# zotya701/OpenCL_Path_tracer

Measured on AMD Instinct MI355X. Metric: Msamples/s (whole node) at 1920x1080, 8-bounce Cornell box, higher is better.
Workload: dtype f32

## Files before the change

### opencl_path_tracer_amd/csrc/pt_builder.cpp

```cpp
#include "pt_context.hpp"

namespace ptamd {

struct RefOrder {
    const std::vector<pt_triangle>& tris;
    std::vector<int32_t>& rank;
    int32_t& next_rank;
    bool degenerate = false;

    struct Range { int32_t begin, end, depth; };

    static int32_t split(const Range& r, int32_t* idx, int32_t* tmp, const float* cx, const float* cy, const float* cz) {
        const int32_t n = r.end - r.begin;
        if (n <= 6) return 0;
        int32_t* ix = idx + r.begin;
        float mx = cx[ix[0]], my = cy[ix[0]], mz = cz[ix[0]];
        for (int32_t i = 1; i < n; ++i) {
            mx = mx + cx[ix[i]];
            my = my + cy[ix[i]];
            mz = mz + cz[ix[i]];
        }
        const float m[3] = {mx / (float)(unsigned long)n, my / (float)(unsigned long)n, mz / (float)(unsigned long)n};
        const float* c[3] = {cx, cy, cz};
        int axis = r.depth % 3;
// ... 978 lines not shown
                    else {
                        const int32_t first = (~ref) >> 3, count = ((~ref) & 7) + 1;
                        good = good && first >= nf && first + count <= n;
                    }
                }
            }
            if (!good) ok.store(false);
        });
        if (!ok.load()) { drop(); return fail(ctx, PT_EHIP, "internal: the device SAH builder returned a malformed tree"); }
    }
    (void)hipFree(r.d_orig);
    r.d_orig = nullptr;
    ctx->host_packets_stale = true;
    ctx->bvh_depth = sah ? r.depth : r.depth + 1;
    ctx->n_flat = nf;
    clk.lap("download + list in front");
    const bool retopped = !sah && sah_top_rebuild(ctx, ctx->lbvh_cluster);
    clk.lap("SAH top over clusters");
    bool wide_done = false;
    int rc = plan_node_placement(ctx, retopped ? nullptr : r.d_nodes, &wide_done);
    clk.lap("node placement + 4-wide nodes");
    if (rc != PT_OK) { drop(); return rc; }
    if (retopped) ctx->bvh_depth = ctx->interior_depth + 1;
    if (ctx->d_tris) (void)hipFree(ctx->d_tris);
    if (ctx->d_meta) (void)hipFree(ctx->d_meta);
    ctx->d_tris = r.d_tris;
    ctx->d_meta = r.d_meta;
    if (retopped) {
        (void)hipFree(r.d_nodes);
        if ((rc = upload_vec(ctx, &ctx->d_nodes, ctx->nodes.data(), sizeof(Node64) * ctx->nodes.size())) != PT_OK) return rc;
    } else {
        if (ctx->d_nodes) (void)hipFree(ctx->d_nodes);
        ctx->d_nodes = r.d_nodes;
        if (ctx->treelet_nodes > 0) PT_HIP(ctx, hipMemcpy(ctx->d_nodes, ctx->nodes.data(), sizeof(Node64) * ctx->nodes.size(), hipMemcpyHostToDevice));
    }
    if (!wide_done && (rc = upload_vec(ctx, &ctx->d_nodes4, ctx->nodes4.data(), sizeof(Node4q) * ctx->nodes4.size())) != PT_OK) return rc;
    if ((rc = alloc_stack_overflow(ctx)) != PT_OK) return rc;
    clk.lap("uploads");
    *done = true;
    return PT_OK;
}

static void compute_cost_boxes(pt_context* ctx) { compute_cost_boxes_impl(ctx); }

int pt_upload_triangles(pt_context* ctx) {
    if (!ctx) return PT_EINVAL;
// ... 8 lines not shown
        int rcd = build_on_device(ctx, &done);
        if (rcd != PT_OK) return rcd;
        if (done) {
            compute_cost_boxes(ctx);
            ctx->bvh_build_ms = std::chrono::duration<double, std::milli>(std::chrono::steady_clock::now() - t0).count();
            ctx->bvh_on_device = 1;
            ctx->tris_uploaded = true;
            return PT_OK;
        }
    }
    ctx->bvh_on_device = 0;
    ctx->host_packets_stale = false;
    int rc = build_and_pack(ctx);
    if (rc != PT_OK) return rc;
    PhaseClock clk("pt_upload_triangles");
    if ((rc = plan_node_placement(ctx)) != PT_OK) return rc;
    clk.lap("node placement + 4-wide nodes");
    ctx->bvh_build_ms = std::chrono::duration<double, std::milli>(std::chrono::steady_clock::now() - t0).count();
    if (ctx->has_device) {
        PT_HIP(ctx, hipSetDevice(ctx->device));
        if ((rc = upload_vec(ctx, &ctx->d_nodes, ctx->nodes.data(), sizeof(Node64) * ctx->nodes.size())) != PT_OK) return rc;
        if ((rc = upload_vec(ctx, &ctx->d_nodes4, ctx->nodes4.data(), sizeof(Node4q) * ctx->nodes4.size())) != PT_OK) return rc;
        if ((rc = alloc_stack_overflow(ctx)) != PT_OK) return rc;
        if ((rc = upload_vec(ctx, &ctx->d_tris, ctx->packets.data(), sizeof(TriPacket) * ctx->packets.size())) != PT_OK) return rc;
        if ((rc = upload_vec(ctx, &ctx->d_meta, ctx->meta.data(), sizeof(TriMeta) * ctx->meta.size())) != PT_OK) return rc;
        clk.lap("device allocations + copies");
    }
    ctx->tris_uploaded = true;
    return PT_OK;
}


}
```

### opencl_path_tracer_amd/csrc/pt_context.hpp

```cpp
#pragma once

#include "pt_internal.hpp"

#include <algorithm>
#include <atomic>
#include <chrono>
#include <cmath>
#include <condition_variable>
#include <functional>
#include <mutex>
#include <cstdio>
#include <cstring>
#include <limits>
#include <memory>
#include <numeric>
#include <queue>
#include <thread>

using namespace ptamd;

namespace ptamd {
struct EventPair {
    hipEvent_t a = nullptr, b = nullptr;
};
// ... 23 lines not shown
    bool tris_uploaded = false, mats_uploaded = false;

    std::vector<Node64> nodes;
    std::vector<Node4q> nodes4;
    int wide_pending = 0;
    std::vector<TriPacket> packets;
    bool host_packets_stale = false;
    std::vector<TriMeta> meta;
    std::vector<int32_t> orig;
    int bvh_depth = 0;
    int interior_depth = 0;
    int n_flat = 0;
    int n_fbox = 0;
    uint8_t fbox_rep[32] = {};
    uint32_t fbox_mask[32] = {};

    float4* d_nodes = nullptr;
    float4* d_nodes4 = nullptr;
    uint32_t* d_stack_ovf = nullptr;
    size_t stack_ovf_lanes = 0;
    float4* d_tris = nullptr;
    TriMeta* d_meta = nullptr;
    pt_material* d_mats = nullptr;
    int32_t* d_rnds = nullptr;
    float4* d_colors = nullptr;
    pt_ray* d_rays = nullptr;
    float4* d_ldr = nullptr;
    unsigned long long* d_stats = nullptr;
    float4* d_wf_state = nullptr;
    int32_t* d_wf_queues = nullptr;
    std::vector<float> cost_boxes;
    uint32_t* d_wf_counters = nullptr;
    hipStream_t wf_stream[kWfMaxChains] = {};
    hipEvent_t wf_event[kWfMaxChains] = {};
    int poll_timeout_ms = 10000;
    int debug_stall_tile = -1;
    bool counters_suspect = false;
    bool launched_since_check = false;
    int wf_streams = -1;
    bool own_rnds = true, own_colors = true;
    hipStream_t stream = nullptr;

    int32_t current_sample = 0;

    int variant = 0;
    int lds_scene = 2;
// ... 199 lines not shown
};

template <class F>
void parallel_for(size_t n, size_t grain, int threads, F fn) {
    const size_t nt = std::min<size_t>((size_t)std::max(threads, 1), (n + grain - 1) / std::max<size_t>(grain, 1));
    if (nt <= 1) { fn((size_t)0, n); return; }
    const size_t per = (n + nt - 1) / nt;
    HostPool::get().run(nt, (int)nt, [&](size_t k) {
        const size_t b = k * per, e = std::min(n, b + per);
        if (b < e) fn(b, e);
    });
}
int deepest_interior_node(const std::vector<Node64>& nodes);
int reindex_treelet(std::vector<Node64>& nodes, int interior_depth, int want);

int32_t count_local_rows(int32_t H, int32_t rank, int32_t world, int32_t rb);
int wide_stack_entries(int pending);
int stack_entries_for(int interior_depth);
bool whole_tree_fits_lds(size_t n_nodes, size_t n_tris, int interior_depth, int n_flat);
int plan_node_placement(pt_context* ctx, const float4* d_bvh2 = nullptr, bool* wide_on_device = nullptr);
int alloc_stack_overflow(pt_context* ctx);
int seed_upload(pt_context* ctx, const int32_t* global_seeds);
void fill_params(const pt_context* ctx, const pt_camera* cam, RenderParams* p);
int check_ready(pt_context* ctx, const pt_camera* cam);
int time_begin(pt_context* ctx, EventPair** ep);
int time_end(pt_context* ctx, EventPair* ep);
int time_collect(pt_context* ctx);
int sync_and_check(pt_context* ctx);
inline int32_t local_tiles(const pt_context* c) { return ((c->W + 7) / 8) * ((c->local_rows + 7) / 8); }
template <class T>
int upload_vec(pt_context* ctx, T** dptr, const void* src, size_t bytes) {
    if (*dptr) { PT_HIP(ctx, hipFree(*dptr)); *dptr = nullptr; }
    PT_HIP(ctx, hipMalloc((void**)dptr, std::max<size_t>(bytes, 64)));
    if (bytes < 64) PT_HIP(ctx, hipMemset(*dptr, 0, 64));
    if (bytes) PT_HIP(ctx, hipMemcpy(*dptr, src, bytes, hipMemcpyHostToDevice));
    return PT_OK;
}


}
```

### opencl_path_tracer_amd/csrc/pt_device.hpp

```cpp
#pragma once

#include "pt_internal.hpp"

#include <algorithm>

#ifndef PT_GLOBAL_SLAB_FMA
#define PT_GLOBAL_SLAB_FMA 1
#endif
#ifndef PT_WIDE_STEP_V1
#define PT_WIDE_STEP_V1 0
#endif
#ifndef PT_PHASE_SWITCH_GLOBAL
#define PT_PHASE_SWITCH_GLOBAL 1
#endif
#ifndef PT_PHASE_SWITCH_LDS
#define PT_PHASE_SWITCH_LDS 1
#endif
#ifndef PT_WIDE_PREDICATED_STORES
#define PT_WIDE_PREDICATED_STORES 1
#endif

namespace ptamd {

struct f3 {
// ... 716 lines not shown
        }
    }
    template <bool COUNT>
    PT_DEV void leaf_step(const SceneView& sv, WorkCount* wc) {
        const int popped = stack_get(sv, tos);
        const int v = leaf_bits(cur);
        const int first = v >> 3, count = (v & 7) + 1;
        for (int j = 0; j < count; ++j) tri_step<COUNT>(sv, first + j, wc);
        cur = popped;
        tos -= stride;
    }
};

template <int MODE, bool COUNT>
PT_DEV int closest_hit(const SceneView& sv, f3 P, f3 D, const LaneStack<typename StackOf<MODE>::type> stk, float* t_out, WorkCount* wc) {
    Trav<MODE> tr;
    tr.begin(P, D, stk);
    tr.template flat_pass<COUNT>(sv, wc);
    while (!tr.done()) tr.template round<COUNT>(sv, wc);
    *t_out = tr.best_t;
    return tr.best;
}

template <bool SK>
PT_DEV f3 diffuse_direction(f3 N, float rnd1, float rnd2) {
    const float E = 0.001f;
    const bool yaxis = __builtin_fabsf(N.x) <= E && __builtin_fabsf(N.z) <= E;
    const float other = yaxis ? N.y : N.x;
    const float l2 = fmaf_(N.z, N.z, other * other);
    float rl, r, z;
    if (wave_all(rsqrt_window(l2) && rnd1 >= kSqrtWindowLo && rnd1 < 1.0f)) {
        rl = rsqrt_core(l2);
        r = sqrt_core(rnd1);
        z = sqrt_core(1.0f - rnd1);
    } else {
        rl = 1.0f / __builtin_sqrtf(l2);
        r = __builtin_sqrtf(rnd1);
        z = __builtin_sqrtf(1.0f - rnd1);
    }
    const f3 Z = yaxis ? mk(0.0f, -N.z * rl, N.y * rl) : mk(-N.z * rl, 0.0f, N.x * rl);
    const f3 X = cross3(N, Z);
    const float theta = (float)(6.283185307179586 * (double)rnd2);
    float sn, cs;
    spec_sincos<SK>(theta, &sn, &cs);
    const float x = r * cs, y = r * sn;
    f3 d = X * x;
    d = madd(N, z, d);
    d = madd(Z, y, d);
    return d;
}

PT_DEV f3 fresnel(f3 F0, f3 N, f3 D) {
    const float cosa = __builtin_fabsf(dot3(N, D));
    const float p5 = spec_pow5(1.0f - cosa);
    return mk(fmaf_(1.0f - F0.x, p5, F0.x), fmaf_(1.0f - F0.y, p5, F0.y), fmaf_(1.0f - F0.z, p5, F0.z));
}

struct PathRegs {
    f3 fL, fB, fS, fR, color;
    PT_DEV void reset() {
        fL = mk(1.f, 1.f, 1.f);
        fB = fL;
        fS = fL;
        fR = fL;
        color = mk(0.f, 0.f, 0.f);
    }
    PT_DEV f3 L() const { return fL; }
    PT_DEV f3 B() const { return fB; }
    PT_DEV f3 S() const { return fS; }
    PT_DEV f3 R() const { return fR; }
    PT_DEV f3 C() const { return color; }
    PT_DEV void setL(f3 v) { fL = v; }
    PT_DEV void setB(f3 v) { fB = v; }
    PT_DEV void setS(f3 v) { fS = v; }
    PT_DEV void setR(f3 v) { fR = v; }
    PT_DEV void setC(f3 v) { color = v; }
};

struct NoShadeHook {
    static constexpr bool active = false;
};

template <bool SK, class ST, class HOOK = NoShadeHook>
PT_DEV void shade_hit(f3& rP, f3& rD, ST& st, int& seed, bool& inside, const RenderParams& p, const float4* tris, const TriMeta* meta, int ti, float t,
                      HOOK* hook = nullptr) {
    const float4 c = tris[ti * 3 + 2];
    f3 N = mk(c.y, c.z, c.w);
    const f3 hp = madd(rD, t, rP);
    const pt_material* __restrict__ m = &p.mats[meta[ti].mati];
    const int type = m->type;
    if (p.iterations == 1) st.setC(ldf3(m->kd) + ldf3(m->emission));
    if (dot3(rD, N) > 0.0f) N = -N;
    const bool lobe = type == 0 || type == 3, spec = type == 1 || type == 2;
    f3 dnew = rD;
    float side = 0.001f;
    float inten = 0.0f;
    float wb = 1.0f;
    if (lobe) {
        inten = max0(dot3(-rD, N));
        if constexpr (HOOK::active) {
            if (type == 3) wb = hook->emitter_weight(ti, t, inten, rD);
            hook->light_sample(st, p, m, type, N, hp);
        }
        const float rnd1 = lcg_rand(seed), rnd2 = lcg_rand(seed);
        dnew = diffuse_direction<SK>(N, rnd1, rnd2);
    } else if (spec) {
        const f3 oldD = rD;
        const f3 F0 = ldf3(m->F0);
        const f3 F = fresnel(F0, N, oldD);
        dnew = oldD - (N * dot3(N, oldD)) * 2.0f;
        if (type == 2) {
            float n = m->n;
            if (inside) n = 1.0f / n;
            const float rnd = lcg_rand(seed);
            const float cosa = dot3(-oldD, N);
            const float disc = 1.0f - (fmaf_(-cosa, cosa, 1.0f) / n) / n;
            const float prob = ((F.x + F.y) + F.z) / 3.0f;
            const bool refr = disc > 0.0f && rnd > prob;
            if (refr) {
                const f3 dn = mk(oldD.x / n, oldD.y / n, oldD.z / n);
                dnew = madd(N, cosa / n - sqrt_rn(disc), dn);
                const float k = 1.0f / (1.0f - prob);
                st.setR((st.R() * mk(1.0f - F.x, 1.0f - F.y, 1.0f - F.z)) * k);
                inside = !inside;
                side = -0.001f;
            } else {
                const float k = 1.0f / prob;
                st.setR((st.R() * F) * k);
            }
        } else {
            st.setS(st.S() * F);
        }
    }
    if (lobe || spec) {
        rD = normalize3(dnew);
        rP = madd(N, side, hp);
    }
    if (type == 0) {
        const float idiff = max0(dot3(rD, N));
        st.setL(st.L() * (ldf3(m->kd) * idiff));
        float pw = 1.0f;
        if (!m->_pad) {
            const f3 view = normalize3(ldf3(p.cam.eye) - hp);
            const f3 halfway = normalize3(view + rD);
            const float ispec = max0(dot3(N, halfway));
            pw = spec_pow<SK>(ispec, m->shininess);
        }
        st.setB(st.B() * (ldf3(m->ks) * pw));
    } else if (type == 3) {
        const f3 e = ((ldf3(m->emission) * (st.L() + st.B())) * st.S()) * st.R();
        if constexpr (HOOK::active) st.setC(madd(e * wb, inten, st.C()));
        else st.setC(madd(e, inten, st.C()));
    }
    if constexpr (HOOK::active) hook->end_vertex(lobe, N);
}

PT_DEV f3 running_mean(f3 acc, f3 color, int s) {
    const float cs = (float)s, cs1 = (float)(s + 1);
    return mk(fmaf_(acc.x, cs, color.x) / cs1, fmaf_(acc.y, cs, color.y) / cs1, fmaf_(acc.z, cs, color.z) / cs1);
}

PT_DEV float luminance(f3 c) { return fmaf_(0.0722f, c.z, fmaf_(0.7152f, c.y, 0.2126f * c.x)); }
PT_DEV float running_moment(float m2, f3 color, int s) {
    const float l = luminance(color);
    return fmaf_(m2, (float)s, l * l) / (float)(s + 1);
}


PT_DEV unsigned stage_ref(float slot) {
    const int r = __float_as_int(slot);
    return (unsigned)(r < 0 ? (0x8000 | ~r) : r) & 0xffffu;
// ... 122 lines not shown
```

### opencl_path_tracer_amd/csrc/pt_host.cpp

```cpp
#include "pt_context.hpp"

namespace {
thread_local std::string g_create_error;
}

namespace ptamd {

int fail(pt_context* ctx, int code, const std::string& msg) {
    if (ctx) ctx->err = msg; else g_create_error = msg;
    return code;
}

int host_threads(const pt_context* ctx) {
    const unsigned hw = std::thread::hardware_concurrency();
    return ctx->build_threads > 0 ? ctx->build_threads : (int)std::min(16u, std::max(1u, hw));
}

int fail_ctx(pt_context* ctx, int code, const std::string& msg) { return fail(ctx, code, msg); }
int append_triangles(pt_context* ctx, int64_t n, pt_triangle** tail) {
    if (!ctx || n < 0 || !tail) return PT_EINVAL;
    if ((int64_t)ctx->tris.size() + n > kMaxTriangles) return fail(ctx, PT_EINVAL, "more than 2^26 triangles");
    const size_t old = ctx->tris.size();
    ctx->tris.resize(old + (size_t)n);
    ctx->tris_uploaded = false;
// ... 153 lines not shown
        pt_destroy(ctx);
        return fail(nullptr, rc, msg);
    }
    *out = ctx;
    return PT_OK;
}

int pt_create(int device, int32_t width, int32_t height, pt_context** out) {
    return pt_create_tiled(device, width, height, 0, 1, 8, out);
}

void pt_destroy(pt_context* ctx) {
    if (!ctx) return;
    if (ctx->has_device) {
        (void)hipSetDevice(ctx->device);
        (void)hipDeviceSynchronize();
        for (auto& e : ctx->events) { if (e.a) (void)hipEventDestroy(e.a); if (e.b) (void)hipEventDestroy(e.b); }
        if (ctx->d_nodes) (void)hipFree(ctx->d_nodes);
        if (ctx->d_nodes4) (void)hipFree(ctx->d_nodes4);
        if (ctx->d_stack_ovf) (void)hipFree(ctx->d_stack_ovf);
        if (ctx->d_tris) (void)hipFree(ctx->d_tris);
        if (ctx->d_meta) (void)hipFree(ctx->d_meta);
        if (ctx->d_mats) (void)hipFree(ctx->d_mats);
        if (ctx->d_rays) (void)hipFree(ctx->d_rays);
        if (ctx->d_ldr) (void)hipFree(ctx->d_ldr);
        if (ctx->d_stats) (void)hipFree(ctx->d_stats);
        if (ctx->d_tile_counter) (void)hipFree(ctx->d_tile_counter);
        if (ctx->d_tile_done) (void)hipFree(ctx->d_tile_done);
        if (ctx->d_tile_cost) (void)hipFree(ctx->d_tile_cost);
        if (ctx->d_adapt_snap) (void)hipFree(ctx->d_adapt_snap);
        if (ctx->d_adapt_spp) (void)hipFree(ctx->d_adapt_spp);
        if (ctx->d_adapt_err) (void)hipFree(ctx->d_adapt_err);
        if (ctx->d_adapt_active) (void)hipFree(ctx->d_adapt_active);
        if (ctx->d_adapt_list) (void)hipFree(ctx->d_adapt_list);
        if (ctx->h_adapt_count) (void)hipHostFree(ctx->h_adapt_count);
        if (ctx->d_aov) (void)hipFree(ctx->d_aov);
        if (ctx->d_dn) (void)hipFree(ctx->d_dn);
        if (ctx->d_variance) (void)hipFree(ctx->d_variance);
        if (ctx->d_temporal) (void)hipFree(ctx->d_temporal);
        if (ctx->d_temporal_var) (void)hipFree(ctx->d_temporal_var);
        if (ctx->d_nee_tri) (void)hipFree(ctx->d_nee_tri);
        if (ctx->d_nee_cdf) (void)hipFree(ctx->d_nee_cdf);
        if (ctx->d_nee_pdf_area) (void)hipFree(ctx->d_nee_pdf_area);
        if (ctx->d_env_texels) (void)hipFree(ctx->d_env_texels);
        if (ctx->d_env_row_cdf) (void)hipFree(ctx->d_env_row_cdf);
        if (ctx->d_env_col_cdf) (void)hipFree(ctx->d_env_col_cdf);
// ... 31 lines not shown

int pt_add_triangle(pt_context* ctx, const pt_triangle* t) { return pt_add_triangles(ctx, t, 1); }

int pt_add_triangles(pt_context* ctx, const pt_triangle* t, int64_t n) {
    if (!ctx || (!t && n) || n < 0) return PT_EINVAL;
    if ((int64_t)ctx->tris.size() + n > kMaxTriangles)
        return fail(ctx, PT_EINVAL, "more than 2^26 triangles");
    ctx->tris.insert(ctx->tris.end(), t, t + n);
    ctx->tris_uploaded = false;
    return PT_OK;
}

int pt_upload_materials(pt_context* ctx) {
    if (!ctx) return PT_EINVAL;
    ctx->aov_valid = false;
    ctx->nee_valid = false;
    for (const pt_triangle& t : ctx->tris)
        if (t.mati >= ctx->mats.size()) return fail(ctx, PT_EINVAL, "a triangle references a material index that was never added");
    if (ctx->has_device) {
        PT_HIP(ctx, hipSetDevice(ctx->device));
        std::vector<pt_material> dm(ctx->mats);
        for (pt_material& m : dm)
            m._pad = (m.ks.s[0] == 0.0f && m.ks.s[1] == 0.0f && m.ks.s[2] == 0.0f && std::isfinite(m.shininess) && m.shininess >= 0.0f) ? 1 : 0;
        int rc = upload_vec(ctx, &ctx->d_mats, dm.data(), sizeof(pt_material) * dm.size());
        if (rc != PT_OK) return rc;
    }
    ctx->mats_uploaded = true;
    return PT_OK;
}

int pt_seed_default(pt_context* ctx) {
    PT_NEED_DEVICE(ctx);
    const size_t n = (size_t)ctx->W * (size_t)ctx->H;
    std::vector<int32_t> g(n);
    uint64_t x = 1;
    for (size_t i = 0; i < n; ++i) {
        x = (x * 16807ull) % 2147483647ull;
        g[i] = (int32_t)x;
    }
    return seed_upload(ctx, g.data());
}

int pt_upload_seeds(pt_context* ctx, const int32_t* seeds, int64_t n) {
    PT_NEED_DEVICE(ctx);
    if (!seeds || n != (int64_t)ctx->W * ctx->H) return fail(ctx, PT_EINVAL, "seeds must hold width*height ints (global frame)");
    return seed_upload(ctx, seeds);
}

// ... 887 lines not shown
```

### opencl_path_tracer_amd/csrc/pt_internal.hpp

```cpp
#pragma once

#include <hip/hip_runtime.h>

#include <atomic>
#include <chrono>
#include <cstdint>
#include <cstdio>
#include <cstdlib>
#include <string>
#include <vector>

#include "pt_api.h"

namespace ptamd {

struct Node64 {
    float q[3][4];
    int32_t left, right;
    int32_t pad[2];
};
static_assert(sizeof(Node64) == 64, "Node64 must be 64 B");

struct TriPacket {
    float v[12];
};
static_assert(sizeof(TriPacket) == 48, "TriPacket must be 48 B");

struct TriMeta {
    int32_t rank;
    int32_t mati;
};

struct Node4q {
    float origin[3];
    uint8_t exp[3];
    uint8_t nchild;
    uint32_t qlo_x, qhi_x, qlo_y, qhi_y;
    uint32_t qlo_z, qhi_z;
    uint32_t spare[2];
    int32_t ref[4];
};
static_assert(sizeof(Node4q) == 64, "Node4q must be 64 B");
constexpr int32_t kWideNoChild = ~0;
constexpr int kWideLdsEntries = 20;
bool build_wide_nodes(const std::vector<Node64>& bvh2, std::vector<Node4q>* out, int* max_pending, int threads);

enum : int { kNodesLds = 0, kNodesGlobal = 1, kNodesTreelet = 2, kNodesWide = 3 };

constexpr int64_t kMaxTriangles = (int64_t)1 << 26;

constexpr int64_t kDeviceBuildFrom = 16384;
constexpr int kMaxLeaf = 4;
constexpr int kMaxDepth = 30;
constexpr int kTileCounterError = 16;
// ... 31 lines not shown
    int32_t n_flat;
    int32_t n_fbox;
    uint8_t fbox_rep[32];
    uint32_t fbox_mask[32];
    int32_t node_mode;
    int32_t treelet_nodes;
    int32_t stack_entries;
    uint32_t* stack_ovf;
    int32_t stack_ovf_lanes;
    uint32_t* tile_counter;
    uint32_t poll_ticks;
    int32_t debug_stall_tile;
    int32_t n_tiles;
    int32_t n_taper;
    uint16_t taper_end[kMaxTaperPasses];
    int32_t chunk_spp;
    uint32_t* tile_done;
    int32_t suspend_lanes;
    int32_t node_min_lanes;
    int32_t leaf_min_lanes;
    int32_t migrate_lanes;
    uint32_t* tile_cost;
    const int32_t* tile_list;
    int32_t moments;
};

template <class P>
__host__ __device__ __forceinline__ int global_row(const P& p, int lrow) {
    return ((lrow / p.rows_per_block) * p.world + p.rank) * p.rows_per_block + lrow % p.rows_per_block;
}

constexpr int kWfCounterStride = 8;
constexpr int kWfMaxBounces = 1023;
constexpr int kWfGenRow = 0;
__host__ __device__ inline int wf_row(int bounce) { return bounce == 0 ? kWfGenRow : bounce + 1; }
constexpr int kWfMaxCostBoxes = 8;
constexpr int kWfMaxChains = 8;
constexpr int kWfDefaultChains = 4;
enum : int { kWfL = 0, kWfB = 1, kWfS = 2, kWfR = 3, kWfC = 4, kWfFields = 5, kWfInsideBit = 1 << 5, kWfBZeroBit = 1 << 6 };
struct WfParams {
    RenderParams rp;
    float* sP;
    float4* rsA[2][2];
    float4* rsB[2][2];
    float4* rsC[2][2];
    float2* hit[2];
// ... 76 lines not shown
    return n;
}

struct PhaseClock {
    const char* who;
    const bool on = std::getenv("PTAMD_TRACE") != nullptr;
    std::chrono::steady_clock::time_point t0 = std::chrono::steady_clock::now();
    explicit PhaseClock(const char* w) : who(w) {}
    void lap(const char* what) {
        if (!on) return;
        const auto t1 = std::chrono::steady_clock::now();
        std::fprintf(stderr, "[%s] %-32s %8.1f ms\n", who, what, std::chrono::duration<double, std::milli>(t1 - t0).count());
        t0 = t1;
    }
};

int traversal_block(int node_mode, bool wide_lds_block);
size_t traversal_lds_bytes(const RenderParams& p, int block);
hipError_t launch_gen_ray(const RenderParams& p, hipStream_t stream);
hipError_t launch_trace_ray(const RenderParams& p, const LaunchConfig& lc, hipStream_t stream);
hipError_t launch_render_mega(const RenderParams& p, const LaunchConfig& lc, hipStream_t stream);
hipError_t launch_resolve_reinhard(const float4* colors, float4* out, int64_t n, hipStream_t stream);
hipError_t launch_filt_im(const float4* colors, float4* out, int32_t width, int32_t height, hipStream_t stream);
hipError_t launch_wf_generate(const WfParams& p, hipStream_t stream);
hipError_t launch_wf_intersect(const WfParams& p, int bounce, int cu_count, hipStream_t stream);
hipError_t launch_wf_shade(const WfParams& p, int bounce, hipStream_t stream);
hipError_t launch_adaptive_tiles(const float4* colors, float4* snap, const int32_t* list, int32_t n_list, int32_t width, int32_t rows, int mode,
                                 float threshold, int32_t spp, float* tile_err, int32_t* tile_spp, uint8_t* active, hipStream_t stream);
hipError_t launch_compact_tiles(const uint8_t* active, int32_t n, int32_t* list, int32_t* count, hipStream_t stream);
hipError_t launch_debug_closest_hit(const RenderParams& p, const pt_ray* rays, int64_t n, float* out_t, int32_t* out_tri, int cu_count, hipStream_t stream);
hipError_t launch_debug_math(int fn, unsigned long long first, unsigned long long n, unsigned long long* out, uint32_t* bad, long long bad_cap, int cu_count,
                             hipStream_t stream);
hipError_t launch_aovs(const RenderParams& p, int32_t subpixels, int32_t specular_depth, int64_t npix, float4* albedo_rgbm, float4* normal_depth,
                       int cu_count, hipStream_t stream);
struct AtrousStep {
    int32_t step;
    int32_t demodulate;
    int32_t color_on, normal_on, depth_on;
    float color_scale;
    float sigma_color2, sigma_normal, sigma_depth;
};
hipError_t launch_atrous(const float4* in, float4* out, const float4* albedo, const float4* nd, int32_t W, int32_t H, const AtrousStep& s,
                         bool first, bool last, hipStream_t stream);
struct AtrousVarStep {
    int32_t step;
    int32_t demodulate;
// ... 95 lines not shown
```

### opencl_path_tracer_amd/csrc/pt_kernels.hip

```cpp
#include "pt_device.hpp"


#include <algorithm>

namespace ptamd {

__global__ void __launch_bounds__(256) k_gen_ray(RenderParams p) {
    const PixelId px = pixel_of_thread(p);
    if (px.li < 0) return;
    int seed = p.rnds[px.li];
    const float rnd1 = lcg_rand(seed), rnd2 = lcg_rand(seed);
    f3 P, D;
    camera_get_ray(px.gid, p.cam, rnd1, rnd2, &P, &D);
    p.rnds[px.li] = seed;
    float4* r = reinterpret_cast<float4*>(&p.rays[px.li]);
    r[0] = make_float4(P.x, P.y, P.z, 0.0f);
    r[1] = make_float4(D.x, D.y, D.z, 0.0f);
}

enum : int { kSchedLockstep = 0, kSchedSuspend = 1, kSchedMigrate = 2 };


PT_DEV void fold_sample(const RenderParams& p, int li, f3 color, int s) {
    f3 acc = mk(0.0f, 0.0f, 0.0f);
    float m2 = 0.0f;
    if (s != 0) {
        const float4 c = p.colors[li];
        acc = mk(c.x, c.y, c.z);
        m2 = c.w;
    }
    acc = running_mean(acc, color, s);
    m2 = p.moments ? running_moment(m2, color, s) : 0.0f;
    p.colors[li] = make_float4(acc.x, acc.y, acc.z, m2);
}

template <bool SPLIT, int MODE, bool COUNT, bool LEAN, bool SK>
PT_DEV void render_pixel_lockstep(const RenderParams& p, const SceneView& sv, const LaneStack<typename StackOf<MODE>::type> stk, const PixelId px,
                                  int s_begin, int s_end, unsigned* segs, WorkCount* wc) {
    int seed = p.rnds[px.li];
    f3 acc = mk(0.0f, 0.0f, 0.0f);
    float m2 = 0.0f;
    if (!LEAN && s_begin != 0) {
        const float4 c = p.colors[px.li];
        acc = mk(c.x, c.y, c.z);
// ... 265 lines not shown
            }
            cur_item = -1;
            if (nxt_item < 0 && !no_more) {
                nxt_item = fetch();
                no_more = __builtin_amdgcn_readfirstlane((int)(nxt_item < 0));
                nxt_ready = 0;
            }
            if (nxt_item < 0) break;
            if (!nxt_ready) {
                if (!wait_released(nxt_item)) break;
                if (pass_of(nxt_item) > 0) __builtin_amdgcn_fence(__ATOMIC_ACQUIRE, "agent");
            }
            cur_item = __builtin_amdgcn_readfirstlane(nxt_item);
            cur_end = __builtin_amdgcn_readfirstlane(end_of(nxt_item));
            nxt_item = -1;
            nxt_ready = 0;
            if (on_next) on_next = false;
            else take_pixel(cur_item);
        } else if (__popcll(__ballot(parked && !on_next)) >= p.migrate_lanes) {
            if (nxt_item < 0 && !no_more) {
                nxt_item = fetch();
                no_more = __builtin_amdgcn_readfirstlane((int)(nxt_item < 0));
                nxt_ready = 0;
                nxt_end = __builtin_amdgcn_readfirstlane(end_of(nxt_item));
            }
            if (nxt_item >= 0 && !nxt_ready && released(nxt_item)) {
                if (pass_of(nxt_item) > 0) __builtin_amdgcn_fence(__ATOMIC_ACQUIRE, "agent");
                nxt_ready = 1;
            }
            if (nxt_item >= 0 && nxt_ready && parked && !on_next) {
                on_next = true;
                take_pixel(nxt_item);
            }
        }
        if (!parked && fresh && !traversing) {
            st.reset();
            inside = false;
            const float rnd1 = lcg_rand(seed), rnd2 = lcg_rand(seed);
            camera_get_ray_xy((float)(pxy & 0xffffu), (float)(pxy >> 16), p.cam, rnd1, rnd2, &rP, &rD);
            bounce = 0;
            fresh = false;
        }
        bool finished = !parked;
        if (!parked && (traversing || bounce < p.iterations)) {
            tr.setup(rP, rD);
            if (!traversing) {
                tr.restart(stk);
                tr.template flat_pass<COUNT>(sv, wc);
            }
            for (;;) {
                if (COUNT && first_active_lane()) wc->wrounds++;
                tr.template round<COUNT>(sv, wc);
                const unsigned long long unfinished = __ballot(!tr.done());
                if (unfinished == 0) break;
                if (__popcll(unfinished) <= p.suspend_lanes && __ballot(tr.done()) != 0) break;
            }
            traversing = !tr.done();
            if (traversing) {
                finished = false;
            } else {
                ++my_segs;
                if (tr.best >= 0) {
                    if (COUNT) { if (first_active_lane()) wc->wshade++; count_low(wc, 3); }
                    shade_hit<SK>(rP, rD, st, seed, inside, p, sv.tris, sv.meta, tr.best, tr.best_t);
                    ++bounce;
                    finished = (bounce >= p.iterations);
                }
            }
        }
        samples += (unsigned long long)__popcll(__ballot(finished));
        if (finished) {
            if (LEAN) fold_sample(p, li, st.C(), s);
            else {
                acc = running_mean(acc, st.C(), s);
                if (p.moments) m2 = running_moment(m2, st.C(), s);
            }
            ++s;
            fresh = true;
        }
    }
    {
        unsigned v = my_segs;
        for (int off = 32; off > 0; off >>= 1) v += __shfl_down(v, off, 64);
        *segs_tot += (unsigned)__builtin_amdgcn_readfirstlane((int)v);
        *samples_tot += samples;
    }
    if (COUNT) {
// ... 257 lines not shown
```

### opencl_path_tracer_amd/csrc/pt_launch.cpp

```cpp
#include "pt_context.hpp"

namespace ptamd {

int32_t count_local_rows(int32_t H, int32_t rank, int32_t world, int32_t rb) {
    int32_t n = 0;
    for (int32_t r = 0; r < H; ++r)
        if ((r / rb) % world == rank) ++n;
    return n;
}

int wide_stack_entries(int pending) { return ((pending + 4) + 1) & ~1; }
int stack_entries_for(int interior_depth) { return std::min(kStackEntries, ((interior_depth + 2) + 1) & ~1); }


bool whole_tree_fits_lds(size_t n_nodes, size_t n_tris, int interior_depth, int n_flat) {
    const bool s16 = n_nodes <= 32767 && n_tris <= 4096;
    const size_t block = (size_t)kLdsBlockBase;
    return s16 && (size_t)kLdsNodeBytes * n_nodes + 16 + (size_t)stack_entries_for(interior_depth) * 2 * block + (size_t)n_flat * 100 + 64 <= kLdsPerCu / 2;
}

static void group_flat_boxes(pt_context* ctx) {
    ctx->n_fbox = 0;
    float ext[32][6];
    for (int k = 0; k < ctx->n_flat; ++k) {
// ... 114 lines not shown
        }
    }
    if (!ctx->nodes4.empty() && (p->node_mode == kNodesGlobal || ctx->wide_nodes == 2)) {
        p->node_mode = kNodesWide;
        p->treelet_nodes = 0;
        p->nodes = ctx->d_nodes4;
        p->stack_entries = std::min(ctx->wide_lds_entries, wide_stack_entries(ctx->wide_pending));
        p->stack_ovf = ctx->d_stack_ovf;
        p->stack_ovf_lanes = (int32_t)ctx->stack_ovf_lanes;
    }
    p->tile_counter = nullptr;
    p->poll_ticks = (uint32_t)std::min<int64_t>((int64_t)ctx->poll_timeout_ms * 100000, 0xffffffffll);
    p->debug_stall_tile = ctx->debug_stall_tile;
    p->chunk_spp = 0;
    p->n_taper = 0;
    p->tile_done = nullptr;
    p->n_tiles = ((ctx->W + 7) / 8) * ((ctx->local_rows + 7) / 8);
    p->suspend_lanes = ctx->suspend_lanes >= 0 ? ctx->suspend_lanes : (p->node_mode == kNodesLds ? 16 : 24);
    p->node_min_lanes = ctx->node_min_lanes >= 0 ? ctx->node_min_lanes : (p->node_mode == kNodesLds ? 3 : 6);
    p->leaf_min_lanes = ctx->leaf_min_lanes >= 0 ? ctx->leaf_min_lanes : 4;
    p->migrate_lanes = ctx->migrate_lanes > 0 ? ctx->migrate_lanes : 1;
}

int check_ready(pt_context* ctx, const pt_camera* cam) {
    if (!cam) return fail(ctx, PT_EINVAL, "camera is NULL");
    if (!ctx->tris_uploaded) return fail(ctx, PT_EINVAL, "pt_upload_triangles has not been called");
    if (!ctx->mats_uploaded) return fail(ctx, PT_EINVAL, "pt_upload_materials has not been called");
    if ((int32_t)cam->XM != ctx->W || (int32_t)cam->YM != ctx->H)
        return fail(ctx, PT_EINVAL, "camera XM/YM do not match the context's frame size");
    return PT_OK;
}

int time_begin(pt_context* ctx, EventPair** ep) {
    *ep = nullptr;
    if (!ctx->timing) return PT_OK;
    if (ctx->events_used == ctx->events.size()) {
        EventPair e;
        PT_HIP(ctx, hipEventCreate(&e.a));
        PT_HIP(ctx, hipEventCreate(&e.b));
        ctx->events.push_back(e);
    }
    *ep = &ctx->events[ctx->events_used++];
    PT_HIP(ctx, hipEventRecord((*ep)->a, ctx->stream));
    return PT_OK;
}
int time_end(pt_context* ctx, EventPair* ep) {
// ... 199 lines not shown
            }
        if (ctx->timing && ctx->events_used >= 4096) {
            int rc = time_collect(ctx);
            if (rc != PT_OK) return rc;
        }
    }
    for (int c = 1; c < chains; ++c) {
        PT_HIP(ctx, hipEventRecord(ctx->wf_event[c], ctx->wf_stream[c]));
        PT_HIP(ctx, hipStreamWaitEvent(ctx->stream, ctx->wf_event[c], 0));
    }
    return PT_OK;
}

static int launch_megakernel(pt_context* ctx, RenderParams& p, const int32_t* tile_list, int32_t n_active) {
    int rc = PT_OK;
    const int32_t nsamples = p.nsamples;
    if (tile_list) {
        p.tile_list = tile_list;
        p.n_tiles = n_active;
    }
    const size_t frame_tiles = (size_t)local_tiles(ctx);
    LaunchConfig lc;
    launch_cfg(ctx, p, &lc);
    if (ctx->persistent) {
        if (int rc2 = prepare_work_counter(ctx)) return rc2;
        p.tile_counter = ctx->d_tile_counter;
        const int resident_waves = ptamd_resident_waves(ctx, lc);
        const int auto_chunk = auto_chunk_spp(p.n_tiles, resident_waves, nsamples, lc.schedule, p.node_mode);
        const int chunk = ctx->chunk_spp >= 0 ? ctx->chunk_spp : auto_chunk;
        int n_pass = chunk > 0 ? (int)(((int64_t)nsamples + chunk - 1) / chunk) : 1;
        const int taper = ctx->chunk_taper >= 0 ? ctx->chunk_taper : auto_chunk_taper(nsamples, lc.schedule, p.node_mode);
        if (chunk > 0 && nsamples > chunk && taper > 0 && taper < chunk && nsamples < 65536) {
            std::vector<int> ends;
            int done = 0;
            while (nsamples - done > chunk) { done += chunk; ends.push_back(done); }
            for (int left = nsamples - done; left > 0;) {
                const int take = left >= 2 * taper ? left / 2 : left;
                done += take;
                left -= take;
                ends.push_back(done);
            }
            if ((int)ends.size() <= kMaxTaperPasses) {
                n_pass = p.n_taper = (int)ends.size();
                for (int k = 0; k < n_pass; ++k) p.taper_end[k] = (uint16_t)ends[k];
            }
        }
// ... 200 lines not shown
```

Baseline: 2779.

## Precompute per-triangle shade records with normal, material fields and tangent frames

```diff
diff --git a/opencl_path_tracer_amd/csrc/pt_builder.cpp b/opencl_path_tracer_amd/csrc/pt_builder.cpp
--- a/opencl_path_tracer_amd/csrc/pt_builder.cpp
+++ b/opencl_path_tracer_amd/csrc/pt_builder.cpp
@@ -1024,6 +1024,7 @@
     clk.lap("node placement + 4-wide nodes");
     if (rc != PT_OK) { drop(); return rc; }
     if (retopped) ctx->bvh_depth = ctx->interior_depth + 1;
+    ctx->shaderec_dirty = true;
     if (ctx->d_tris) (void)hipFree(ctx->d_tris);
     if (ctx->d_meta) (void)hipFree(ctx->d_meta);
     ctx->d_tris = r.d_tris;
@@ -1078,6 +1079,7 @@
         if ((rc = upload_vec(ctx, &ctx->d_nodes, ctx->nodes.data(), sizeof(Node64) * ctx->nodes.size())) != PT_OK) return rc;
         if ((rc = upload_vec(ctx, &ctx->d_nodes4, ctx->nodes4.data(), sizeof(Node4q) * ctx->nodes4.size())) != PT_OK) return rc;
         if ((rc = alloc_stack_overflow(ctx)) != PT_OK) return rc;
+        ctx->shaderec_dirty = true;
         if ((rc = upload_vec(ctx, &ctx->d_tris, ctx->packets.data(), sizeof(TriPacket) * ctx->packets.size())) != PT_OK) return rc;
         if ((rc = upload_vec(ctx, &ctx->d_meta, ctx->meta.data(), sizeof(TriMeta) * ctx->meta.size())) != PT_OK) return rc;
         clk.lap("device allocations + copies");
diff --git a/opencl_path_tracer_amd/csrc/pt_context.hpp b/opencl_path_tracer_amd/csrc/pt_context.hpp
--- a/opencl_path_tracer_amd/csrc/pt_context.hpp
+++ b/opencl_path_tracer_amd/csrc/pt_context.hpp
@@ -69,6 +69,10 @@
     float4* d_tris = nullptr;
     TriMeta* d_meta = nullptr;
     pt_material* d_mats = nullptr;
+    ShadeRec* d_shaderec = nullptr;
+    size_t shaderec_cap = 0;
+    bool shaderec_dirty = true;
+    int32_t mats_on_device = 0;
     int32_t* d_rnds = nullptr;
     float4* d_colors = nullptr;
     pt_ray* d_rays = nullptr;
@@ -314,6 +318,7 @@
 int alloc_stack_overflow(pt_context* ctx);
 int seed_upload(pt_context* ctx, const int32_t* global_seeds);
 void fill_params(const pt_context* ctx, const pt_camera* cam, RenderParams* p);
+int ensure_shade_records(pt_context* ctx, RenderParams* p);
 int check_ready(pt_context* ctx, const pt_camera* cam);
 int time_begin(pt_context* ctx, EventPair** ep);
 int time_end(pt_context* ctx, EventPair* ep);
diff --git a/opencl_path_tracer_amd/csrc/pt_device.hpp b/opencl_path_tracer_amd/csrc/pt_device.hpp
--- a/opencl_path_tracer_amd/csrc/pt_device.hpp
+++ b/opencl_path_tracer_amd/csrc/pt_device.hpp
@@ -762,12 +762,36 @@
     return tr.best;
 }
 
+PT_DEV float frame_l2(f3 N, bool* yaxis) {
+    const float E = 0.001f;
+    *yaxis = __builtin_fabsf(N.x) <= E && __builtin_fabsf(N.z) <= E;
+    const float other = *yaxis ? N.y : N.x;
+    return fmaf_(N.z, N.z, other * other);
+}
+PT_DEV void frame_from_rl(f3 N, bool yaxis, float rl, f3* Z, f3* X) {
+    *Z = yaxis ? mk(0.0f, -N.z * rl, N.y * rl) : mk(-N.z * rl, 0.0f, N.x * rl);
+    *X = cross3(N, *Z);
+}
+PT_DEV void tangent_frame(f3 N, f3* Z, f3* X) {
+    bool yaxis;
+    const float l2 = frame_l2(N, &yaxis);
+    frame_from_rl(N, yaxis, rsqrt_rn(l2), Z, X);
+}
+template <bool SK>
+PT_DEV f3 lobe_direction(f3 N, f3 Z, f3 X, float r, float z, float rnd2) {
+    const float theta = (float)(6.283185307179586 * (double)rnd2);
+    float sn, cs;
+    spec_sincos<SK>(theta, &sn, &cs);
+    const float x = r * cs, y = r * sn;
+    f3 d = X * x;
+    d = madd(N, z, d);
+    d = madd(Z, y, d);
+    return d;
+}
 template <bool SK>
 PT_DEV f3 diffuse_direction(f3 N, float rnd1, float rnd2) {
-    const float E = 0.001f;
-    const bool yaxis = __builtin_fabsf(N.x) <= E && __builtin_fabsf(N.z) <= E;
-    const float other = yaxis ? N.y : N.x;
-    const float l2 = fmaf_(N.z, N.z, other * other);
+    bool yaxis;
+    const float l2 = frame_l2(N, &yaxis);
     float rl, r, z;
     if (wave_all(rsqrt_window(l2) && rnd1 >= kSqrtWindowLo && rnd1 < 1.0f)) {
         rl = rsqrt_core(l2);
@@ -778,16 +802,22 @@
         r = __builtin_sqrtf(rnd1);
         z = __builtin_sqrtf(1.0f - rnd1);
     }
-    const f3 Z = yaxis ? mk(0.0f, -N.z * rl, N.y * rl) : mk(-N.z * rl, 0.0f, N.x * rl);
-    const f3 X = cross3(N, Z);
-    const float theta = (float)(6.283185307179586 * (double)rnd2);
-    float sn, cs;
-    spec_sincos<SK>(theta, &sn, &cs);
-    const float x = r * cs, y = r * sn;
-    f3 d = X * x;
-    d = madd(N, z, d);
-    d = madd(Z, y, d);
-    return d;
+    f3 Z, X;
+    frame_from_rl(N, yaxis, rl, &Z, &X);
+    return lobe_direction<SK>(N, Z, X, r, z, rnd2);
+}
+template <bool SK>
+PT_DEV f3 diffuse_direction_rec(f3 N, const float4* frame, float rnd1, float rnd2) {
+    const float4 fa = frame[0], fb = frame[1];
+    float r, z;
+    if (wave_all(rnd1 >= kSqrtWindowLo && rnd1 < 1.0f)) {
+        r = sqrt_core(rnd1);
+        z = sqrt_core(1.0f - rnd1);
+    } else {
+        r = __builtin_sqrtf(rnd1);
+        z = __builtin_sqrtf(1.0f - rnd1);
+    }
+    return lobe_direction<SK>(N, mk(fa.x, fa.y, fa.z), mk(fa.w, fb.x, fb.y), r, z, rnd2);
 }
 
 PT_DEV f3 fresnel(f3 F0, f3 N, f3 D) {
@@ -821,16 +851,35 @@
     static constexpr bool active = false;
 };
 
-template <bool SK, class ST, class HOOK = NoShadeHook>
+template <bool SK, bool REC = false, class ST, class HOOK = NoShadeHook>
 PT_DEV void shade_hit(f3& rP, f3& rD, ST& st, int& seed, bool& inside, const RenderParams& p, const float4* tris, const TriMeta* meta, int ti, float t,
                       HOOK* hook = nullptr) {
-    const float4 c = tris[ti * 3 + 2];
-    f3 N = mk(c.y, c.z, c.w);
+    f3 N, kd;
+    int type;
+    bool plain;
+    const pt_material* __restrict__ m;
+    const float4* rec = nullptr;
+    if constexpr (REC) {
+        rec = p.shaderec + (size_t)ti * (sizeof(ShadeRec) / sizeof(float4));
+        const float4 a = rec[0], b = rec[1];
+        N = mk(a.x, a.y, a.z);
+        type = __float_as_int(a.w);
+        kd = mk(b.x, b.y, b.z);
+        const unsigned mi = (unsigned)__float_as_int(b.w);
+        plain = (mi & kShadeRecPlain) != 0;
+        m = &p.mats[mi & ~kShadeRecPlain];
+    } else {
+        const float4 c = tris[ti * 3 + 2];
+        N = mk(c.y, c.z, c.w);
+        m = &p.mats[meta[ti].mati];
+        type = m->type;
+        kd = mk(0.0f, 0.0f, 0.0f);
+        plain = false;
+    }
     const f3 hp = madd(rD, t, rP);
-    const pt_material* __restrict__ m = &p.mats[meta[ti].mati];
-    const int type = m->type;
-    if (p.iterations == 1) st.setC(ldf3(m->kd) + ldf3(m->emission));
-    if (dot3(rD, N) > 0.0f) N = -N;
+    if (p.iterations == 1) st.setC((REC ? kd : ldf3(m->kd)) + ldf3(m->emission));
+    const bool flip = dot3(rD, N) > 0.0f;
+    if (flip) N = -N;
     const bool lobe = type == 0 || type == 3, spec = type == 1 || type == 2;
     f3 dnew = rD;
     float side = 0.001f;
@@ -843,7 +892,8 @@
             hook->light_sample(st, p, m, type, N, hp);
         }
         const float rnd1 = lcg_rand(seed), rnd2 = lcg_rand(seed);
-        dnew = diffuse_direction<SK>(N, rnd1, rnd2);
+        if constexpr (REC) dnew = diffuse_direction_rec<SK>(N, rec + (flip ? 4 : 2), rnd1, rnd2);
+        else dnew = diffuse_direction<SK>(N, rnd1, rnd2);
     } else if (spec) {
         const f3 oldD = rD;
         const f3 F0 = ldf3(m->F0);
@@ -878,15 +928,19 @@
     }
     if (type == 0) {
         const float idiff = max0(dot3(rD, N));
-        st.setL(st.L() * (ldf3(m->kd) * idiff));
-        float pw = 1.0f;
-        if (!m->_pad) {
-            const f3 view = normalize3(ldf3(p.cam.eye) - hp);
-            const f3 halfway = normalize3(view + rD);
-            const float ispec = max0(dot3(N, halfway));
-            pw = spec_pow<SK>(ispec, m->shininess);
-        }
-        st.setB(st.B() * (ldf3(m->ks) * pw));
+        st.setL(st.L() * ((REC ? kd : ldf3(m->kd)) * idiff));
+        if (REC && plain) {
+            st.setB(st.B() * mk(0.0f, 0.0f, 0.0f));
+        } else {
+            float pw = 1.0f;
+            if (!m->_pad) {
+                const f3 view = normalize3(ldf3(p.cam.eye) - hp);
+                const f3 halfway = normalize3(view + rD);
+                const float ispec = max0(dot3(N, halfway));
+                pw = spec_pow<SK>(ispec, m->shininess);
+            }
+            st.setB(st.B() * (ldf3(m->ks) * pw));
+        }
     } else if (type == 3) {
         const f3 e = ((ldf3(m->emission) * (st.L() + st.B())) * st.S()) * st.R();
         if constexpr (HOOK::active) st.setC(madd(e * wb, inten, st.C()));
diff --git a/opencl_path_tracer_amd/csrc/pt_host.cpp b/opencl_path_tracer_amd/csrc/pt_host.cpp
--- a/opencl_path_tracer_amd/csrc/pt_host.cpp
+++ b/opencl_path_tracer_amd/csrc/pt_host.cpp
@@ -199,6 +199,7 @@
         if (ctx->d_tris) (void)hipFree(ctx->d_tris);
         if (ctx->d_meta) (void)hipFree(ctx->d_meta);
         if (ctx->d_mats) (void)hipFree(ctx->d_mats);
+        if (ctx->d_shaderec) (void)hipFree(ctx->d_shaderec);
         if (ctx->d_rays) (void)hipFree(ctx->d_rays);
         if (ctx->d_ldr) (void)hipFree(ctx->d_ldr);
         if (ctx->d_stats) (void)hipFree(ctx->d_stats);
@@ -276,8 +277,10 @@
         std::vector<pt_material> dm(ctx->mats);
         for (pt_material& m : dm)
             m._pad = (m.ks.s[0] == 0.0f && m.ks.s[1] == 0.0f && m.ks.s[2] == 0.0f && std::isfinite(m.shininess) && m.shininess >= 0.0f) ? 1 : 0;
+        ctx->shaderec_dirty = true;
         int rc = upload_vec(ctx, &ctx->d_mats, dm.data(), sizeof(pt_material) * dm.size());
         if (rc != PT_OK) return rc;
+        ctx->mats_on_device = (int32_t)dm.size();
     }
     ctx->mats_uploaded = true;
     return PT_OK;
diff --git a/opencl_path_tracer_amd/csrc/pt_internal.hpp b/opencl_path_tracer_amd/csrc/pt_internal.hpp
--- a/opencl_path_tracer_amd/csrc/pt_internal.hpp
+++ b/opencl_path_tracer_amd/csrc/pt_internal.hpp
@@ -30,6 +30,18 @@
     int32_t rank;
     int32_t mati;
 };
+
+struct ShadeRec {
+    float N[3];
+    int32_t type;
+    float kd[3];
+    uint32_t mati;
+    float frame[2][8];
+};
+static_assert(sizeof(ShadeRec) == 96, "ShadeRec must be 96 B");
+constexpr uint32_t kShadeRecPlain = 0x80000000u;
+constexpr int32_t kShadeRecNoMaterial = 0x7fffffff;
+constexpr bool shade_records_for(int node_mode) { return node_mode == 0 ; }
 
 struct Node4q {
     float origin[3];
@@ -107,6 +119,7 @@
     int32_t migrate_lanes;
     uint32_t* tile_cost;
     const int32_t* tile_list;
+    const float4* shaderec;
     int32_t moments;
 };
 
@@ -229,6 +242,7 @@
 hipError_t launch_render_mega(const RenderParams& p, const LaunchConfig& lc, hipStream_t stream);
 hipError_t launch_resolve_reinhard(const float4* colors, float4* out, int64_t n, hipStream_t stream);
 hipError_t launch_filt_im(const float4* colors, float4* out, int32_t width, int32_t height, hipStream_t stream);
+hipError_t launch_shade_records(const float4* tris, const TriMeta* meta, const pt_material* mats, int32_t n_mats, int32_t n, ShadeRec* out, hipStream_t stream);
 hipError_t launch_wf_generate(const WfParams& p, hipStream_t stream);
 hipError_t launch_wf_intersect(const WfParams& p, int bounce, int cu_count, hipStream_t stream);
 hipError_t launch_wf_shade(const WfParams& p, int bounce, hipStream_t stream);
diff --git a/opencl_path_tracer_amd/csrc/pt_kernels.hip b/opencl_path_tracer_amd/csrc/pt_kernels.hip
--- a/opencl_path_tracer_amd/csrc/pt_kernels.hip
+++ b/opencl_path_tracer_amd/csrc/pt_kernels.hip
@@ -20,6 +20,8 @@
 
 enum : int { kSchedLockstep = 0, kSchedSuspend = 1, kSchedMigrate = 2 };
 
+template <int MODE>
+constexpr bool kShadeRec = shade_records_for(MODE);
 
 PT_DEV void fold_sample(const RenderParams& p, int li, f3 color, int s) {
     f3 acc = mk(0.0f, 0.0f, 0.0f);
@@ -331,7 +333,7 @@
                 nxt_item = fetch();
                 no_more = __builtin_amdgcn_readfirstlane((int)(nxt_item < 0));
                 nxt_ready = 0;
-                nxt_end = __builtin_amdgcn_readfirstlane(end_of(nxt_item));
+                if (nxt_item >= 0) nxt_end = __builtin_amdgcn_readfirstlane(end_of(nxt_item));
             }
             if (nxt_item >= 0 && !nxt_ready && released(nxt_item)) {
                 if (pass_of(nxt_item) > 0) __builtin_amdgcn_fence(__ATOMIC_ACQUIRE, "agent");
@@ -371,7 +373,7 @@
                 ++my_segs;
                 if (tr.best >= 0) {
                     if (COUNT) { if (first_active_lane()) wc->wshade++; count_low(wc, 3); }
-                    shade_hit<SK>(rP, rD, st, seed, inside, p, sv.tris, sv.meta, tr.best, tr.best_t);
+                    shade_hit<SK, kShadeRec<MODE>>(rP, rD, st, seed, inside, p, sv.tris, sv.meta, tr.best, tr.best_t);
                     ++bounce;
                     finished = (bounce >= p.iterations);
                 }
diff --git a/opencl_path_tracer_amd/csrc/pt_launch.cpp b/opencl_path_tracer_amd/csrc/pt_launch.cpp
--- a/opencl_path_tracer_amd/csrc/pt_launch.cpp
+++ b/opencl_path_tracer_amd/csrc/pt_launch.cpp
@@ -160,6 +160,25 @@
     p->migrate_lanes = ctx->migrate_lanes > 0 ? ctx->migrate_lanes : 1;
 }
 
+int ensure_shade_records(pt_context* ctx, RenderParams* p) {
+    p->shaderec = nullptr;
+    if (!shade_records_for(p->node_mode)) return PT_OK;
+    if (ctx->shaderec_dirty) {
+        const size_t n = ctx->orig.size();
+        if (!ctx->d_shaderec || ctx->shaderec_cap < std::max<size_t>(n, 1)) {
+            if (ctx->d_shaderec) { PT_HIP(ctx, hipFree(ctx->d_shaderec)); ctx->d_shaderec = nullptr; }
+            ctx->shaderec_cap = 0;
+            PT_HIP(ctx, hipMalloc((void**)&ctx->d_shaderec, sizeof(ShadeRec) * std::max<size_t>(n, 1)));
+            ctx->shaderec_cap = std::max<size_t>(n, 1);
+        }
+        if (n == 0) PT_HIP(ctx, hipMemsetAsync(ctx->d_shaderec, 0, sizeof(ShadeRec), ctx->stream));
+        PT_HIP(ctx, launch_shade_records(ctx->d_tris, ctx->d_meta, ctx->d_mats, ctx->mats_on_device, (int32_t)n, ctx->d_shaderec, ctx->stream));
+        ctx->shaderec_dirty = false;
+    }
+    p->shaderec = reinterpret_cast<const float4*>(ctx->d_shaderec);
+    return PT_OK;
+}
+
 int check_ready(pt_context* ctx, const pt_camera* cam) {
     if (!cam) return fail(ctx, PT_EINVAL, "camera is NULL");
     if (!ctx->tris_uploaded) return fail(ctx, PT_EINVAL, "pt_upload_triangles has not been called");
@@ -405,6 +424,7 @@
     const size_t frame_tiles = (size_t)local_tiles(ctx);
     LaunchConfig lc;
     launch_cfg(ctx, p, &lc);
+    if (lc.schedule == 2 && ctx->persistent && (rc = ensure_shade_records(ctx, &p)) != PT_OK) return rc;
     if (ctx->persistent) {
         if (int rc2 = prepare_work_counter(ctx)) return rc2;
         p.tile_counter = ctx->d_tile_counter;
diff --git a/opencl_path_tracer_amd/csrc/pt_shaderec.hip b/opencl_path_tracer_amd/csrc/pt_shaderec.hip
--- /dev/null
+++ b/opencl_path_tracer_amd/csrc/pt_shaderec.hip
@@ -0,0 +1,46 @@
+#include "pt_device.hpp"
+
+namespace ptamd {
+
+__global__ void __launch_bounds__(256) k_shade_records(const float4* tris, const TriMeta* meta, const pt_material* mats, int n_mats, int n, ShadeRec* out) {
+    const int ti = blockIdx.x * blockDim.x + threadIdx.x;
+    if (ti >= n) return;
+    const float4 c = tris[(size_t)ti * 3 + 2];
+    const f3 N = mk(c.y, c.z, c.w);
+    const int mati = meta[ti].mati;
+    ShadeRec r;
+    r.N[0] = N.x;
+    r.N[1] = N.y;
+    r.N[2] = N.z;
+    r.type = kShadeRecNoMaterial;
+    r.kd[0] = r.kd[1] = r.kd[2] = 0.0f;
+    r.mati = (uint32_t)mati & ~kShadeRecPlain;
+    if (mati >= 0 && mati < n_mats) {
+        const pt_material* m = &mats[mati];
+        r.type = m->type;
+        for (int k = 0; k < 3; ++k) r.kd[k] = m->kd.s[k];
+        const bool ks_pos0 = __float_as_int(m->ks.s[0]) == 0 && __float_as_int(m->ks.s[1]) == 0 && __float_as_int(m->ks.s[2]) == 0;
+        if (m->_pad && ks_pos0) r.mati |= kShadeRecPlain;
+    }
+    for (int o = 0; o < 2; ++o) {
+        f3 Z, X;
+        tangent_frame(o == 0 ? N : -N, &Z, &X);
+        r.frame[o][0] = Z.x;
+        r.frame[o][1] = Z.y;
+        r.frame[o][2] = Z.z;
+        r.frame[o][3] = X.x;
+        r.frame[o][4] = X.y;
+        r.frame[o][5] = X.z;
+        r.frame[o][6] = 0.0f;
+        r.frame[o][7] = 0.0f;
+    }
+    out[ti] = r;
+}
+
+hipError_t launch_shade_records(const float4* tris, const TriMeta* meta, const pt_material* mats, int32_t n_mats, int32_t n, ShadeRec* out, hipStream_t stream) {
+    if (n <= 0) return hipSuccess;
+    hipLaunchKernelGGL(k_shade_records, dim3((unsigned)((n + 255) / 256)), dim3(256), 0, stream, tris, meta, mats, (int)n_mats, (int)n, out);
+    return hipGetLastError();
+}
+
+}
```

Measured after the change: 2837 (median of 6 runs). 1.02x the previous value.
